# erwincoumans/tiny-differentiable-simulator

Measured on NVIDIA H100. Metric: env-steps/sec (N parallel sims), higher is better.
Workload: dtype f32 (ABA, factorisation, PGS) + f64 (kinematics, inertias, CRBA, Jacobians, LCP rhs)

## Files before the change

### tiny-differentiable-simulator_b200/csrc/tds_capi.cu

```cuda
#include <cuda_runtime.h>
#include <stdio.h>
#include <stdlib.h>
#include <string.h>

#include <algorithm>
#include <mutex>
#include <string>
#include <vector>

#include "tds_b200.h"
#include "tds_b200_model.h"
#include "tds_model.h"
#include "tds_types.h"
#include "tds_team.h"
#include "tds_tape.cuh"
#include "tds_host_io.h"

extern "C" int tds_launch_stept(const TeamModel* TM, const TeamLink* tl_dev, const DevModel* M, const SimParams* P,
                                const EnvParams* E, const StepIO* io, int mode, int use_pd, int precision,
                                char* gscratch, int use_smem, cudaStream_t stream);
extern "C" size_t tds_stept_tile_bytes(const TeamModel* TM);
extern "C" unsigned long long tds_stepr_table_owner(int dev);
extern "C" int tds_launch_stepr(const TeamModel* TM, const TeamLink* tl_host, unsigned long long token, const DevModel* M,
                                const SimParams* P, const EnvParams* E, const StepIO* io, int mode, int use_pd,
// ... 289 lines not shown
  float* S = stats + (size_t)(2 * n_obs + o) * ns + e;
  const float c = *cnt + 1.f;
  if (c == 1.f) { *mean = x; *S = 0.f; }
  else { const float m0 = *mean, m1 = m0 + (x - m0) / c; *S += (x - m0) * (x - m1); *mean = m1; }
  *cnt = c;
}
__global__ void ars_perturb_kernel(const float* __restrict__ w, const float* __restrict__ deltas, float scale,
                                   float* __restrict__ params, int n, int ns) {
  const int e = blockIdx.x * blockDim.x + threadIdx.x;
  const int p = blockIdx.y;
  if (e >= n) return;
  params[(size_t)p * ns + e] = w[p] + scale * deltas[(size_t)p * ns + e];
}
__global__ void ars_update_kernel(float* __restrict__ w, const float* __restrict__ deltas, const float* __restrict__ r_pos,
                                  const float* __restrict__ r_neg, float delta_std, float step_size, int n, int ns) {
  __shared__ float red[256];
  const int p = blockIdx.x;
  float acc = 0.f;
  for (int e = threadIdx.x; e < n; e += blockDim.x) acc += (r_pos[e] - r_neg[e]) * deltas[(size_t)p * ns + e];
  red[threadIdx.x] = acc;
  __syncthreads();
  for (int s = blockDim.x / 2; s > 0; s >>= 1) {
    if ((int)threadIdx.x < s) red[threadIdx.x] += red[threadIdx.x + s];
    __syncthreads();
  }
  if (threadIdx.x == 0) w[p] += step_size * (red[0] * delta_std / (float)n);
}
__global__ void rollout_init_kernel(float* sticky, float* total, int* steps, int n) {
  const int e = blockIdx.x * blockDim.x + threadIdx.x;
  if (e < n) { sticky[e] = 0.f; total[e] = 0.f; steps[e] = 0; }
}

}

struct tds_b200_sim {
  int device = 0;
  int n = 0, ns = 0;
  DevModel dm[3];
  DevModel dm_ad;
  char* jac_scratch = nullptr; size_t jac_scratch_bytes = 0;
  double* jac_dev = nullptr; size_t jac_dev_bytes = 0;
  int tape_cap = 4096;
  char* vjp_buf = nullptr; size_t vjp_buf_bytes = 0;
  int* vjp_flag = nullptr;
  double* vjp_g = nullptr; size_t vjp_g_bytes = 0;
  double* jvp_dev = nullptr; size_t jvp_dev_bytes = 0;
  DevModel dm_m;
  double* mass_dev = nullptr; size_t mass_dev_bytes = 0;
  ParMap par;
  double* par_dev = nullptr; size_t par_dev_bytes = 0;
  bool smem_ok[3] = {false, false, false};
  bool smem_ok_w[3] = {false, false, false};
  int kernel = 4;
  int kernel_req = 4;
  bool spec_ok = false;
  int spec_idx = -1;
  std::vector<double> model;
  bool smem_ok_r[3] = {false, false, false};
  unsigned long long table_token = 0;
  bool team_ok = false;
  bool smem_ok_t[3] = {false, false, false};
  TeamModel tm[3];
  std::vector<TeamLink> team_table;
  TeamLink* team_dev = nullptr;
  int warps_per_block[3] = {1, 1, 1};
  DevVisuals vis;
  SimParams P;
  EnvParams E;
  int precision_req = TDS_B200_PREC_AUTO;
  int precision = TDS_B200_PREC_F64;
  int n_tau = 0, n_points = 0;
  ContactCandTable cand;
  int *c_count = nullptr, *c_links = nullptr, *c_cand = nullptr;
  size_t c_count_bytes = 0, c_links_bytes = 0, c_cand_bytes = 0;
  float *q = nullptr, *qd = nullptr, *act = nullptr, *qdd = nullptr, *reward = nullptr, *done = nullptr;
  float *cdist = nullptr, *link_xf = nullptr;
  char* scratch = nullptr;
  size_t scratch_bytes = 0;
  void* stage_dev = nullptr;
  size_t stage_dev_bytes = 0;
  cudaStream_t stream = nullptr;
  int max_smem_optin = 0;
  long long* phase_clk = nullptr;
  float *rq = nullptr, *rqd = nullptr, *zero_act = nullptr, *pol_act = nullptr, *sticky = nullptr, *r_total = nullptr, *pol_params = nullptr;
  int *act_qidx = nullptr, *r_steps = nullptr;
  float* obs_stats = nullptr;
  bool act_qidx_valid = false;
  size_t pol_params_bytes = 0;
  const float* io_act_aos = nullptr; float* io_obs_aos = nullptr; float* io_obs_tail = nullptr;
  const void* zc_key[4] = {nullptr, nullptr, nullptr, nullptr};
  void* zc_dev[4] = {nullptr, nullptr, nullptr, nullptr};
  bool zc_ok = false;
  unsigned zc_calls = 0;
  const void* g_key[4] = {nullptr, nullptr, nullptr, nullptr};
  int g_seen = 0;
  cudaGraphExec_t g_exec = nullptr;
};

static void drop_host_graph(tds_b200_sim* s) {
  if (s->g_exec) { cudaGraphExecDestroy(s->g_exec); s->g_exec = nullptr; }
  s->g_seen = 0;
  s->g_key[0] = s->g_key[1] = s->g_key[2] = s->g_key[3] = nullptr;
}

static bool is_pinned(const void* p) {
  if (!p) return true;
  cudaPointerAttributes a;
  if (cudaPointerGetAttributes(&a, p) != cudaSuccess) { cudaGetLastError(); return false; }
  return a.type == cudaMemoryTypeHost;
}

static int ensure_stage(tds_b200_sim* s, size_t bytes) {
  if (bytes > s->stage_dev_bytes) {
    drop_host_graph(s);
    CUDA_TRY(grow_dev(&s->stage_dev, &s->stage_dev_bytes, bytes));
  }
  return 0;
}

static int ensure_scratch(tds_b200_sim* s, int prec) {
  const int words = s->dm[prec].w_total > s->dm[prec].x_total ? s->dm[prec].w_total : s->dm[prec].x_total;
  CUDA_TRY(grow_dev(&s->scratch, &s->scratch_bytes, (size_t)words * 4 * s->ns));
  return 0;
}

static int enter_derivative_host(tds_b200_sim* s) {
  CUDA_TRY(cudaSetDevice(s->device));
  CUDA_TRY(cudaDeviceSynchronize());
  return 0;
}


static int put_state(tds_b200_sim* s, const double* src, int dim, float* dst) {
  if (dim == 0) return 0;
  CUDA_TRY(cudaMemcpyAsync(s->stage_dev, src, sizeof(double) * s->n * dim, cudaMemcpyHostToDevice, s->stream));
  aos_to_soa_kernel<double><<<(s->n + 127) / 128, 128, 0, s->stream>>>((const double*)s->stage_dev, dim, 0, dst, dim, s->n, s->ns);
  return 0;
}

static int put_q(tds_b200_sim* s, const double* q) {
  const DevModel& M = s->dm[0];
  const size_t rows = (size_t)(M.n_q > M.n_qd ? M.n_q : M.n_qd) + s->n_points + 1;
  if (int rc = ensure_stage(s, sizeof(double) * s->n * rows)) return rc;
  return put_state(s, q, M.n_q, s->q);
}

static int put_step_inputs(tds_b200_sim* s, int use_pd, const double* q, const double* qd, const double* tau_or_action) {
  const int n_in = use_pd ? s->E.n_act : s->n_tau;
  int rc = put_q(s, q);
  if (!rc) rc = put_state(s, qd, s->dm[0].n_qd, s->qd);
  if (rc) return rc;
  if (tau_or_action) return put_state(s, tau_or_action, n_in, s->act);
  CUDA_TRY(cudaMemsetAsync(s->act, 0, sizeof(float) * s->ns * (n_in > 0 ? n_in : 1), s->stream));
  return 0;
}

static int get_state(tds_b200_sim* s, const float* src, int dim, double* dst) {
  if (dim == 0 || !dst) return 0;
  if (int rc = ensure_stage(s, sizeof(double) * s->n * dim)) return rc;
  soa_to_aos_kernel<double><<<(s->n + 127) / 128, 128, 0, s->stream>>>(src, (double*)s->stage_dev, dim, 0, dim, s->n, s->ns);
  CUDA_TRY(cudaMemcpyAsync(dst, s->stage_dev, sizeof(double) * s->n * dim, cudaMemcpyDeviceToHost, s->stream));
  CUDA_TRY(cudaStreamSynchronize(s->stream));
  return 0;
}

static int rebuild_team(tds_b200_sim* s) {
// ... 180 lines not shown
  E.auto_reset = s->E.auto_reset;
  memcpy(E.reset_q, s->E.reset_q, sizeof(E.reset_q));
  s->E = E;
  s->act_qidx_valid = false;
  return rebuild_team(s);
}

int tds_b200_set_auto_reset(tds_b200_sim* s, int enable, const double* reset_q) {
  if (!s) return -1;
  const DevModel& M = s->dm[0];
  if (enable && !reset_q) { set_err("auto-reset needs a reset pose"); return -1; }
  drop_host_graph(s);
  s->E.auto_reset = enable ? 1 : 0;
  if (reset_q)
    for (int k = 0; k < M.n_q; ++k) s->E.reset_q[k] = (float)reset_q[k];
  return 0;
}

int tds_b200_set_precision(tds_b200_sim* s, int precision) {
  if (!s || precision < TDS_B200_PREC_AUTO || precision > 2) return -1;
  drop_host_graph(s);
  s->precision_req = precision;
  s->precision = precision != TDS_B200_PREC_AUTO ? precision : (s->spec_ok ? TDS_B200_PREC_MIXED : TDS_B200_PREC_F64);
  return 0;
}

int tds_b200_param_count(const tds_b200_sim* s) { return s ? tds_param_count(&s->dm[0]) : -1; }

static int set_physical_params(tds_b200_sim* s, int k, const int* ids, const double* values, bool device, void* stream) {
  if (!s) return -1;
  if (k > 0 && !values) { set_err("physical params: null values"); return -1; }
  ParMap pm;
  const char* err = nullptr;
  if (tds_build_par_map(&s->dm[0], k, ids, &pm, &err)) { set_err(std::string("physical params: ") + err); return -2; }
  CUDA_TRY(cudaSetDevice(s->device));
  const bool same_ids = memcmp(&pm, &s->par, sizeof(pm)) == 0;
  if (!same_ids) drop_host_graph(s);
  if (k == 0) {
    s->par = pm;
    return 0;
  }
  const size_t bytes = sizeof(double) * (size_t)k * s->ns;
  if (bytes > s->par_dev_bytes) {
    drop_host_graph(s);
    CUDA_TRY(grow_dev(&s->par_dev, &s->par_dev_bytes, bytes));
    CUDA_TRY(cudaMemset(s->par_dev, 0, bytes));
  }
  if (device) {
    CUDA_TRY(cudaMemcpyAsync(s->par_dev, values, bytes, cudaMemcpyDeviceToDevice, (cudaStream_t)stream));
  } else {
    CUDA_TRY(cudaDeviceSynchronize());
    CUDA_TRY(put_rows(s->par_dev, values, k, s->n, s->ns, s->stream));
    CUDA_TRY(cudaDeviceSynchronize());
  }
  s->par = pm;
  return 0;
}

int tds_b200_set_physical_params_device(tds_b200_sim* s, int k, const int* ids, const double* values, void* stream) {
  return set_physical_params(s, k, ids, values, true, stream);
}

int tds_b200_set_physical_params_host(tds_b200_sim* s, int k, const int* ids, const double* values) {
  return set_physical_params(s, k, ids, values, false, nullptr);
}

int tds_b200_get_dims(const tds_b200_sim* s, int dims[8]) {
  if (!s) return -1;
  const DevModel& M = s->dm[0];
  dims[0] = s->n; dims[1] = s->ns; dims[2] = M.n_q; dims[3] = M.n_qd; dims[4] = s->n_tau; dims[5] = M.n_links;
  dims[6] = s->n_points; dims[7] = s->E.n_act;
  return 0;
}

int tds_b200_step_device(tds_b200_sim* s, int mode, int use_pd, const float* q_in, const float* qd_in,
                         const float* tau_or_action, float* q_out, float* qd_out, float* qdd_out, float* reward,
                         float* done, float* contact_dist, float* link_xf, void* stream) {
  if (!s) return -1;
  const int p = s->precision;
  StepIO io;
  io.q_in = q_in; io.qd_in = qd_in; io.tau_in = tau_or_action;
  io.q_out = q_out; io.qd_out = qd_out; io.qdd_out = qdd_out;
  io.reward = reward; io.done = done; io.contact_dist = contact_dist; io.link_xf = link_xf;
  io.phase_clk = s->phase_clk;
  io.act_aos = s->io_act_aos; io.obs_aos = s->io_obs_aos; io.obs_tail = s->io_obs_tail;
  io.jac = nullptr; io.jac_n_in = 0; io.jac_dir0 = 0;
  io.n = s->n; io.n_stride = s->ns;
  if (use_pd && s->E.n_act == 0) { set_err("use_pd without tds_b200_set_env"); return -3; }
  int kern = s->kernel_req;
  if (s->dm[0].world_only || mode == 3 || s->P.contact_model != 0 || s->par.n > 0) kern = 1;
  if (kern == 4 && !(s->spec_ok && tds_spec_smem_bytes(s->spec_idx, p) <= (size_t)s->max_smem_optin)) kern = 3;
  if (kern == 4) {
    s->kernel = kern;
    static const int solo = getenv("TDS_B200_DEBUG_SOLO") ? 256 : 0;
    int rcs = tds_launch_step_spec(s->spec_idx, &s->P, &s->E, &io, mode | solo, use_pd, p, (cudaStream_t)stream);
    if (rcs) set_err(std::string("specialised step launch: ") + cudaGetErrorString((cudaError_t)rcs));
    return rcs;
  }
  if (kern == 3 && !(s->team_ok && s->smem_ok_r[p])) kern = 2;
  if (kern == 2 && !s->team_ok) kern = 1;
  s->kernel = kern;
  if (kern == 3) {
    int rcr = tds_launch_stepr(&s->tm[p], s->team_table.data(), s->table_token, &s->dm[p], &s->P, &s->E, &io, mode, use_pd, p,
                               nullptr, 1, (cudaStream_t)stream);
    if (rcr) set_err(std::string("role-warp step launch: ") + cudaGetErrorString((cudaError_t)rcr));
    return rcr;
  }
  if (kern == 2) {
    const int use_smem_t = s->smem_ok_t[p] ? 1 : 0;
    if (!use_smem_t)
      CUDA_TRY(grow_dev(&s->scratch, &s->scratch_bytes, tds_stept_tile_bytes(&s->tm[p]) * ((s->n + (32 / TDS_TEAM_T) - 1) / (32 / TDS_TEAM_T))));
    int rct = tds_launch_stept(&s->tm[p], s->team_dev, &s->dm[p], &s->P, &s->E, &io, mode, use_pd, p, s->scratch, use_smem_t,
                               (cudaStream_t)stream);
    if (rct) set_err(std::string("team step launch: ") + cudaGetErrorString((cudaError_t)rct));
    return rct;
  }
  const int use_smem = s->smem_ok_w[p] ? 1 : 0;
  if (!use_smem) { int rc = ensure_scratch(s, p); if (rc) return rc; }
  ParMap pm = s->par;
  pm.values = s->par_dev; pm.grad = nullptr;
  int rc = s->par.n > 0
      ? tds_launch_stepw_par(&s->dm[p], &s->P, &s->E, &io, &pm, mode, use_pd, p, s->scratch, use_smem, s->warps_per_block[p],
                             (cudaStream_t)stream)
      : tds_launch_stepw(&s->dm[p], &s->P, &s->E, &io, mode, use_pd, p, s->scratch, use_smem, s->warps_per_block[p], (cudaStream_t)stream);
  if (rc) set_err(std::string("step launch: ") + cudaGetErrorString((cudaError_t)rc));
  return rc;
}

int tds_b200_jacobian_dims(const tds_b200_sim* s, int mode, int use_pd, int dims[2]) {
  if (!s || !dims) return -1;
  const DevModel& M = s->dm[0];
  dims[0] = mode == TDS_B200_MODE_FD ? M.n_qd : M.n_q + M.n_qd;
  dims[1] = M.n_q + M.n_qd + (use_pd ? s->E.n_act + 3 : s->n_tau);
  return 0;
}

struct JvpTangents { const double* t_in; const double* t_par; int m; bool mass = false; const TdsKinCall* kin = nullptr; };

static size_t lane_arena_bytes(const tds_b200_sim* s, const DevModel& M) {
  return (size_t)(s->n + 31) / 32 * (size_t)M.x_total * 32 * 4;
}

static int dir_chunk(const tds_b200_sim* s) {
  const size_t chunk = ((size_t)2 << 30) / lane_arena_bytes(s, s->dm_ad);
  return (int)(chunk < 1 ? 1 : (chunk > 65535 ? 65535 : chunk));
}

static int jacobian_run(tds_b200_sim* s, int mode, int use_pd, const float* q, const float* qd, const float* tau_or_action,
                        double* jac, void* stream, bool params, const JvpTangents* jv = nullptr) {
  int dims[2];
  tds_b200_jacobian_dims(s, mode, use_pd, dims);
  const int n_dirs = jv ? jv->m : (params ? s->par.n : dims[1]), dir_base = (params && !jv) ? dims[1] : 0;
  StepIO io;
  memset(&io, 0, sizeof(io));
  io.q_in = q; io.qd_in = qd; io.tau_in = tau_or_action;
  io.jac = jac; io.jac_n_in = n_dirs;
  io.n = s->n; io.n_stride = s->ns;
  ParMap pmv = s->par;
  pmv.values = s->par_dev; pmv.grad = nullptr;
  const ParMap* pm = s->par.n > 0 ? &pmv : nullptr;
  const int chunk = std::min(dir_chunk(s), n_dirs);
  CUDA_TRY(grow_dev(&s->jac_scratch, &s->jac_scratch_bytes, lane_arena_bytes(s, s->dm_ad) * chunk));
  for (int d0 = 0; d0 < n_dirs; d0 += chunk) {
    io.jac_dir0 = dir_base + d0;
    const int nd = n_dirs - d0 < chunk ? n_dirs - d0 : chunk;
    int rc = (jv && jv->kin) ? tds_launch_kin_jvp(&s->dm_ad, &io, jv->kin, jv->t_in, jv->m, nd, s->jac_scratch, (cudaStream_t)stream)
           : (jv && jv->mass) ? tds_launch_mass_jvp(&s->dm_ad, &io, pm, jv->t_in, jv->t_par, jv->m, nd, s->jac_scratch, (cudaStream_t)stream)
// ... 726 lines not shown
  return 0;
}

int tds_b200_env_set_obs_stats(tds_b200_sim* s, float* stats) {
  if (!s) return -1;
  s->obs_stats = stats;
  return 0;
}

int tds_b200_env_rollout_device(tds_b200_sim* s, const float* policy, int n_params, int rollout_length, float shift,
                                float* total_rewards, int* steps, void* stream) {
  if (!s || !policy || !total_rewards || !steps) return -1;
  if (s->E.n_act == 0) { set_err("rollout without tds_b200_set_env"); return -3; }
  const DevModel& M = s->dm[0];
  if (n_params != s->E.n_act * (M.n_q + M.n_qd) + s->E.n_act) { set_err("policy size must be n_act * (n_q + n_qd) + n_act"); return -2; }
  CUDA_TRY(cudaSetDevice(s->device));
  int rc = ensure_env_layer(s);
  if (rc) return rc;
  cudaStream_t sm = stream ? (cudaStream_t)stream : s->stream;
  const int T = 128, B = (s->n + T - 1) / T;
  rollout_init_kernel<<<B, T, 0, sm>>>(s->sticky, total_rewards, steps, s->n);
  const int saved_auto = s->E.auto_reset;
  s->E.auto_reset = 0;
  for (int r = 0; r < rollout_length && rc == 0; ++r) {
    policy_linear_kernel<<<dim3(B, s->E.n_act), T, 0, sm>>>(s->q, s->qd, policy, s->pol_act, M.n_q, M.n_qd, s->E.n_act, s->n, s->ns);
    if (s->obs_stats) obs_stat_push_kernel<<<dim3(B, M.n_q + M.n_qd), T, 0, sm>>>(s->q, s->qd, s->obs_stats, M.n_q, M.n_qd, s->n, s->ns);
    rc = tds_b200_step_device(s, TDS_B200_MODE_FULL, 1, s->q, s->qd, s->pol_act, s->q, s->qd, nullptr, s->reward, s->done, nullptr,
                              nullptr, sm);
    rollout_accum_kernel<<<B, T, 0, sm>>>(s->reward, s->done, shift, s->sticky, total_rewards, steps, s->n);
  }
  s->E.auto_reset = saved_auto;
  if (rc) return rc;
  CUDA_TRY(cudaGetLastError());
  return 0;
}

int tds_b200_env_rollout_host(tds_b200_sim* s, const double* policy, int n_params, int rollout_length, double shift,
                              const double* noise, double noise_amp, unsigned long long seed, int settle_steps,
                              double* total_rewards, int* steps) {
  if (!s || !policy) return -1;
  CUDA_TRY(cudaSetDevice(s->device));
  int rc = ensure_env_layer(s);
  if (rc) return rc;
  const int n = s->n, ns = s->ns, na = s->E.n_act;
  cudaStream_t sm = s->stream;
  const size_t rows = (size_t)n_params > (size_t)na ? (size_t)n_params : (size_t)na;
  CUDA_TRY(grow_dev(&s->pol_params, &s->pol_params_bytes, sizeof(float) * rows * ns));
  rc = ensure_stage(s, sizeof(double) * (size_t)n * rows);
  if (!rc && noise) rc = put_state(s, noise, na, s->pol_params);
  if (!rc) rc = tds_b200_env_reset_device(s, nullptr, noise ? s->pol_params : nullptr, (float)noise_amp, seed, settle_steps, sm);
  if (!rc) rc = put_state(s, policy, n_params, s->pol_params);
  if (!rc) rc = tds_b200_env_rollout_device(s, s->pol_params, n_params, rollout_length, (float)shift, s->r_total, s->r_steps, sm);
  if (rc) return rc;
  std::vector<float> tot(n);
  CUDA_TRY(cudaMemcpyAsync(tot.data(), s->r_total, sizeof(float) * n, cudaMemcpyDeviceToHost, sm));
  if (steps) CUDA_TRY(cudaMemcpyAsync(steps, s->r_steps, sizeof(int) * n, cudaMemcpyDeviceToHost, sm));
  CUDA_TRY(cudaStreamSynchronize(sm));
  if (total_rewards) for (int i = 0; i < n; ++i) total_rewards[i] = (double)tot[i];
  return 0;
}

int tds_b200_get_precision(const tds_b200_sim* s) { return s ? s->precision : -1; }

const char* tds_b200_kernel_name(const tds_b200_sim* s) {
  static const char* names[5] = {"", "tds_stepw_kernel (common frame, lane per environment)",
                                 "tds_stept_kernel (lane team per environment)", "tds_stepr_kernel (warp per tree role)",
                                 "tds_step_spec_kernel (warp per tree role, model-specialised)"};
  return (s && s->kernel >= 0 && s->kernel <= 4) ? names[s->kernel] : "";
}

int tds_b200_debug_phase_clocks(tds_b200_sim* s, int enable, long long* out_host, int cap_warps) {
  if (!s) return -1;
  const int nw = s->ns / (32 / TDS_TEAM_T);
  if (enable && !s->phase_clk) {
    CUDA_TRY(cudaMalloc((void**)&s->phase_clk, sizeof(long long) * 16 * nw));
    CUDA_TRY(cudaMemset(s->phase_clk, 0, sizeof(long long) * 16 * nw));
  }
  if (out_host && s->phase_clk) {
    CUDA_TRY(cudaDeviceSynchronize());
    CUDA_TRY(cudaMemcpy(out_host, s->phase_clk, sizeof(long long) * 16 * (nw < cap_warps ? nw : cap_warps), cudaMemcpyDeviceToHost));
  }
  if (!enable && s->phase_clk) { cudaFree(s->phase_clk); s->phase_clk = nullptr; }
  return nw;
}

void* tds_b200_stream(tds_b200_sim* s) { return s ? (void*)s->stream : nullptr; }
float* tds_b200_env_q(tds_b200_sim* s) { return s ? s->q : nullptr; }
float* tds_b200_env_qd(tds_b200_sim* s) { return s ? s->qd : nullptr; }

int tds_b200_env_step_host(tds_b200_sim* s, const float* actions, float* obs, float* rewards, float* dones) {
  if (!s || !actions) return -1;
  CUDA_TRY(cudaSetDevice(s->device));
  const DevModel& M = s->dm[0];
  const int n = s->n, ns = s->ns, na = s->E.n_act, nobs = M.n_q + M.n_qd;
  const size_t in_b = sizeof(float) * (size_t)n * na, obs_b = sizeof(float) * (size_t)n * nobs;
  const bool packed = obs && rewards == obs + (size_t)n * nobs && dones == rewards + n;
  int rc = ensure_stage(s, in_b + obs_b + sizeof(float) * 2 * (size_t)n);
  if (rc) return rc;
  float* d_in = (float*)s->stage_dev;
  float* d_obs = (float*)((char*)s->stage_dev + in_b);
  cudaStream_t sm = s->stream;
  const int T = 128, B = (n + T - 1) / T;
  const bool direct = s->kernel_req == 4 && s->spec_ok && s->P.contact_model == 0 && s->par.n == 0 && tds_spec_smem_bytes(s->spec_idx, s->precision) <= (size_t)s->max_smem_optin;
  auto enqueue = [&]() -> int {
    CUDA_TRY(cudaMemcpyAsync(d_in, actions, in_b, cudaMemcpyHostToDevice, sm));
    if (direct) {
      s->io_act_aos = d_in; s->io_obs_aos = obs ? d_obs : nullptr; s->io_obs_tail = (obs && packed) ? d_obs + (size_t)n * nobs : nullptr;
    } else aos_to_soa_kernel<float><<<B, T, 0, sm>>>(d_in, na, 0, s->act, na, n, ns);
    int r = tds_b200_step_device(s, TDS_B200_MODE_FULL, 1, s->q, s->qd, s->act, s->q, s->qd, nullptr, s->reward, s->done,
                                 nullptr, nullptr, sm);
    s->io_act_aos = nullptr; s->io_obs_aos = nullptr; s->io_obs_tail = nullptr;
    if (r) return r;
    if (obs && direct) {
      CUDA_TRY(cudaMemcpyAsync(obs, d_obs, obs_b + (packed ? sizeof(float) * 2 * (size_t)n : 0), cudaMemcpyDeviceToHost, sm));
    } else if (obs) {
      pack_env_out_kernel<<<B, T, 0, sm>>>(s->q, s->qd, s->reward, s->done, d_obs, M.n_q, M.n_qd, n, ns, packed ? 1 : 0);
      CUDA_TRY(cudaMemcpyAsync(obs, d_obs, obs_b + (packed ? sizeof(float) * 2 * (size_t)n : 0), cudaMemcpyDeviceToHost, sm));
    }
    if (!packed) {
      if (rewards) CUDA_TRY(cudaMemcpyAsync(rewards, s->reward, sizeof(float) * n, cudaMemcpyDeviceToHost, sm));
      if (dones) CUDA_TRY(cudaMemcpyAsync(dones, s->done, sizeof(float) * n, cudaMemcpyDeviceToHost, sm));
    }
    return 0;
  };
  static const bool no_zero_copy = getenv("TDS_B200_NO_ZEROCOPY") != nullptr;
  if (direct && !s->phase_clk && !no_zero_copy) {
    void *da = nullptr, *dob = nullptr, *dr = nullptr, *dd = nullptr;
    bool ok;
    if ((++s->zc_calls & 63u) != 0 && s->zc_key[0] == actions && s->zc_key[1] == obs && s->zc_key[2] == rewards && s->zc_key[3] == dones) {
      ok = s->zc_ok;
      da = s->zc_dev[0]; dob = s->zc_dev[1]; dr = s->zc_dev[2]; dd = s->zc_dev[3];
    } else {
      ok = is_pinned(actions) && is_pinned(obs) && is_pinned(rewards) && is_pinned(dones);
      ok = ok && cudaHostGetDevicePointer(&da, (void*)actions, 0) == cudaSuccess;
      if (ok && obs) ok = cudaHostGetDevicePointer(&dob, obs, 0) == cudaSuccess;
      if (ok && rewards) ok = cudaHostGetDevicePointer(&dr, rewards, 0) == cudaSuccess;
      if (ok && dones) ok = cudaHostGetDevicePointer(&dd, dones, 0) == cudaSuccess;
      if (!ok) cudaGetLastError();
      s->zc_key[0] = actions; s->zc_key[1] = obs; s->zc_key[2] = rewards; s->zc_key[3] = dones;
      s->zc_dev[0] = da; s->zc_dev[1] = dob; s->zc_dev[2] = dr; s->zc_dev[3] = dd;
      s->zc_ok = ok;
    }
    if (ok) {
      s->io_act_aos = (const float*)da; s->io_obs_aos = (float*)dob; s->io_obs_tail = nullptr;
      rc = tds_b200_step_device(s, TDS_B200_MODE_FULL, 1, s->q, s->qd, s->act, s->q, s->qd, nullptr, dr ? (float*)dr : s->reward,
                                dd ? (float*)dd : s->done, nullptr, nullptr, sm);
      s->io_act_aos = nullptr; s->io_obs_aos = nullptr;
      if (rc) return rc;
      CUDA_TRY(cudaStreamSynchronize(sm));
      CUDA_TRY(cudaGetLastError());
      return 0;
    }
  }
  const void* key[4] = {actions, obs, rewards, dones};
  const bool same = s->g_key[0] == key[0] && s->g_key[1] == key[1] && s->g_key[2] == key[2] && s->g_key[3] == key[3];
  if (s->g_exec && s->kernel == 3 && tds_stepr_table_owner(s->device) != s->table_token) drop_host_graph(s);
  if (same && s->g_exec) {
    CUDA_TRY(cudaGraphLaunch(s->g_exec, sm));
  } else if (same && s->g_seen >= 2 && !s->phase_clk && is_pinned(actions) && is_pinned(obs) && is_pinned(rewards) && is_pinned(dones)) {
    cudaGraph_t g = nullptr;
    CUDA_TRY(cudaStreamBeginCapture(sm, cudaStreamCaptureModeThreadLocal));
    rc = enqueue();
    cudaError_t ce = cudaStreamEndCapture(sm, &g);
    if (rc || ce != cudaSuccess) {
      if (g) cudaGraphDestroy(g);
      cudaGetLastError();
// ... 214 lines not shown
```

### tiny-differentiable-simulator_b200/csrc/tds_steps.cu

```cuda
#include <cuda_runtime.h>
#include <stdlib.h>

#include "tds_wcommon.cuh"
#include "tds_team.h"
#include "generated/spec_laikago.h"
#include "generated/spec_ant.h"

namespace tdss {
using namespace tds;
using namespace tdsw;

#ifndef TDS_DENSE_MAX_CAND
#define TDS_DENSE_MAX_CAND 8
#endif
constexpr int TT = TDS_TEAM_T;
constexpr int ST = 32;

template <int V> struct IC { static constexpr int value = V; };
#define CI(...) (IC<(__VA_ARGS__)>::value)
#define CD(...) ([]() { constexpr double cd_v_ = (__VA_ARGS__); return cd_v_; }())
#define CDOT3(ax, ay, az, v)                                                                                            \
  ([&]() {                                                                                                              \
    using T_ = decltype((v).x);                                                                                         \
    constexpr double a_ = (ax), b_ = (ay), c_ = (az);                                                                   \
// ... 145 lines not shown
  }
  return true;
}
template <class SP> __host__ __device__ constexpr bool trunk_direct() {
  if (!trunk_is_chain<SP>() || SP::FLOATING) return false;
  for (int k = 0; k < SP::N_TRUNK; ++k) {
    if (SP::L_FLAGS[0][k] & TDS_LF_FIXED) return false;
    if (SP::L_SD[0][k][0] != 0.0 || SP::L_SD[0][k][1] != 0.0) return false;
    if (k < SP::N_TRUNK - 1 && (!trunk_massless<SP>(k) || SP::L_ACC[0][k] >= 0 || SP::L_XW[0][k] >= 0)) return false;
  }
  return true;
}
template <class SP> constexpr TrunkTab<SP> make_trunk() {
  TrunkTab<SP> t{};
  for (int k = 0; k < SP::N_TRUNK; ++k) {
    const double* b = SP::L_RBIC[0][k];
    t.fixed[k] = (SP::L_FLAGS[0][k] & TDS_LF_FIXED) ? 1 : 0;
    t.massless[k] = (b[0] == 0.0 && b[4] == 0.0 && b[5] == 0.0 && b[6] == 0.0 && b[7] == 0.0 && b[8] == 0.0 && b[9] == 0.0) ? 1 : 0;
    t.rbi_slot[k] = trunk_rbi_slot<SP>(k);
    t.acc[k] = SP::L_ACC[0][k]; t.ldof[k] = SP::L_LDOF[0][k]; t.qdidx[k] = SP::L_QDIDX[0][k]; t.xw[k] = SP::L_XW[0][k];
    t.sd[k][0] = (float)SP::L_SD[0][k][0]; t.sd[k][1] = (float)SP::L_SD[0][k][1];
  }
  return t;
}
template <class SP> __device__ const TrunkTab<SP>& trunk_tab();

template <class SP> struct CandTab {
  static constexpr int NC = SP::N_CAND > 0 ? SP::N_CAND : 1;
  int owner[NC], own[NC];
};
template <class SP> constexpr CandTab<SP> make_cand() {
  CandTab<SP> t{};
  for (int g = 0; g < SP::N_CAND; ++g) {
    t.owner[g] = SP::CAND_OWNER[g];
    t.own[g] = (SP::CAND_OWNER[g] == 0 && SP::CAND_LPT[g] < Cls<SP>::n_pts_trunk()) ? 0 : 1;
  }
  return t;
}
template <class SP> __device__ const CandTab<SP>& cand_tab();

template <class SP, typename RA, typename RC, typename RS> struct Lay {
  static constexpr int RAW = sizeof(RA) / 4, RCW = sizeof(RC) / 4, RSW = sizeof(RS) / 4;
  static constexpr int NTD = SP::N_TD, NTRI = NTD * (NTD + 1) / 2, NOD = SP::N_OD_MAX;
  static constexpr int O = 0;
  static constexpr int RB = O + 4 * RCW;
  static constexpr int XWW = ev(12 * RCW + 12 * RAW);
  static constexpr int XW = RB + 10 * RCW;
  static constexpr int TS = XW + (SP::N_XW_TEAM + 1) * XWW;
  static constexpr int TLW = ev(14 * RAW);
  static constexpr int TL = TS + SP::N_TRUNK * 6 * RCW;
  static constexpr int TLR = ev(TL + SP::N_TRUNK * TLW);
  static constexpr int TKS = ev(TLR + trunk_rbi_slot<SP>(SP::N_TRUNK) * 10 * RCW);
  static constexpr int TQD = ev(TKS + 3 * SP::N_TRUNK);
  static constexpr int ACC_IC = ev(27 * RAW);
  static constexpr int ACCW = ev(ACC_IC + 10 * RCW);
  static constexpr int ACC = ev(TQD + NTD);
  static constexpr int PW = ev(NTRI * RSW);
  static constexpr int CONW = ev((3 * (NOD + NTD) + 9) * RSW);
  static constexpr int ACC_SZ = cmax(cmax(TT * cmax(SP::N_ATT, 1) * ACCW, TT * PW), cmax(SP::N_CAND, 1) * CONW);
  static constexpr int LT = ACC + ACC_SZ;
  static constexpr int CON = ACC;
  static constexpr int ZT = ev(LT + NTRI * RSW);
  static constexpr int WO = ev(ZT + NTD * RSW);
  static constexpr int ASTG = ev(WO + TT * NOD * RSW);
  static constexpr int XS = ev(ASTG + SP::N_ACT);
  static constexpr int FLG = ev(XS + (SP::N_CAND > TDS_DENSE_MAX_CAND ? 3 * SP::N_CAND * RSW : 0));
  static constexpr int SHARED = ev(FLG + 2 * TT + 2);
  static constexpr int PRIV = ev(cmax(SP::KMAX - SP::N_TRUNK, 1) * 10 * RCW);
  static constexpr int TOTAL = SHARED + TT * PRIV;
};

template <typename T> TDS_D T* sp(char* base, int lane, int word) {
  return (sizeof(T) == 4) ? ((T*)base) + (size_t)word * ST + lane : ((T*)base) + (size_t)(word >> 1) * ST + lane;
}
template <typename T> TDS_D T negz() { return T(-0.0); }
template <typename T> TDS_D Abi<T> abi_nz() {
  Abi<T> a; const T z = negz<T>();
  a.I = {z, z, z, z, z, z}; a.M = a.I;
  a.H.xx = a.H.xy = a.H.xz = a.H.yx = a.H.yy = a.H.yz = a.H.zx = a.H.zy = a.H.zz = z;
  return a;
}
template <typename T> TDS_D Sv<T> sv_nz() { Sv<T> s; const T z = negz<T>(); s.top = v3<T>(z, z, z); s.bot = s.top; return s; }
template <typename T> TDS_D Rbi<T> rbi_nz() { Rbi<T> r; const T z = negz<T>(); r.m = z; r.h = v3<T>(z, z, z); r.I = {z, z, z, z, z, z}; return r; }

template <class SP, typename RA, typename RC, typename RS, int VAR>
TDS_D void tile_body(char* const smem, const SimParams& P, const EnvParams& E, const StepIO& io, const int mode, const int use_pd,
                     const int role, const int tile, const int tid) {
  using L = Lay<SP, RA, RC, RS>;
  using C = Cls<SP>;
  static_assert(C::uniform(), "the subtrees of the model are not one structural class (use the table-driven kernel)");
  constexpr bool XOUT = VAR == 0, HOSTIO = VAR == 2;
  constexpr int RAW = L::RAW, RCW = L::RCW;
  constexpr int NT = SP::N_TRUNK, NTD = SP::N_TD, NLOC = SP::N_LOC[0];
  constexpr int NOD = SP::N_OD[0], NODA = cmax(NOD, 1), NTDA = cmax(NTD, 1), NTRI = L::NTRI, NTRIA = cmax(NTRI, 1);
  constexpr int NPO = C::n_pts_own(), NPOA = cmax(NPO, 1), NPTR = C::n_pts_trunk(), NPTRA = cmax(NPTR, 1);
  constexpr int NACCA = cmax(SP::N_ACC, 1), NXLA = cmax(SP::N_XW_LANE, 1), NATT = cmax(SP::N_ATT, 1);
  constexpr bool FLOAT = SP::FLOATING != 0;
  const int lane = tid & 31;
  const int env = tile * 32 + lane;
  const bool live = env < io.n;
  const int e = live ? env : io.n - 1;
  const int ns = io.n_stride;
  const LegTab<SP>& LG = leg_tab<SP>(role);
  char* const priv = smem + (size_t)(L::SHARED + role * L::PRIV) * ST * 4;
  int phase_id = 0;
#define TDSS_PHASE() do { if (io.phase_clk && lane == 0 && tile * 32 < io.n_stride) io.phase_clk[((size_t)tile * TT + role) * 16 + phase_id] = clock64(); ++phase_id; } while (0)
#define TDSS_STAMP(slot) do { if (io.phase_clk && lane == 0 && tile * 32 < io.n_stride) io.phase_clk[((size_t)tile * TT + role) * 16 + (slot)] = clock64(); } while (0)
  TDSS_PHASE();
  auto xw_rc = [&](int slot) { return sp<RC>(smem, lane, L::XW + slot * L::XWW); };
  auto xw_ra = [&](int slot) { return sp<RA>(smem, lane, L::XW + slot * L::XWW + 12 * RCW); };
  auto tl_rbi_slot = [&](int slot) { return sp<RC>(smem, lane, L::TLR + slot * 10 * RCW); };
  auto tl_u = [&](int k) { return sp<RA>(smem, lane, L::TL + k * L::TLW); };
  auto tl_v = [&](int k) { return sp<RA>(smem, lane, L::TL + k * L::TLW + 8 * RAW); };
  auto ts_S = [&](int k) { return sp<RC>(smem, lane, L::TS + k * 6 * RCW); };
  float* const tqd = sp<float>(smem, lane, L::TQD);
  unsigned* const flg = sp<unsigned>(smem, lane, L::FLG);

  float qv[SP::KMAX], qdv[SP::KMAX], tauv[SP::KMAX];
  float bq[7], bqd[6];
  sfor<NT, NLOC>([&](auto Kc) {
    constexpr int k = decltype(Kc)::value;
    if constexpr (!(C::flags(k) & TDS_LF_FIXED)) {
      qv[k] = io.q_in[(size_t)LG.qidx[k - NT] * ns + e];
      qdv[k] = io.qd_in[(size_t)LG.qdidx[k - NT] * ns + e];
      tauv[k] = 0.f;
    }
  });
  if (role == 0) {
    sfor<0, NT>([&](auto Kc) {
      constexpr int k = decltype(Kc)::value;
      if constexpr (!(SP::L_FLAGS[0][k] & TDS_LF_FIXED)) {
        qv[k] = io.q_in[(size_t)CI(SP::L_QIDX[0][k]) * ns + e];
        qdv[k] = io.qd_in[(size_t)CI(SP::L_QDIDX[0][k]) * ns + e];
        tauv[k] = 0.f;
      }
    });
    if constexpr (FLOAT) {
#pragma unroll
      for (int k = 0; k < 7; ++k) bq[k] = io.q_in[(size_t)k * ns + e];
#pragma unroll
      for (int k = 0; k < 6; ++k) bqd[k] = io.qd_in[(size_t)k * ns + e];
    }
  }
  constexpr int NACT_TILE = 32 * SP::N_ACT, AREG = (NACT_TILE + 32 * TT - 1) / (32 * TT);
  float areg[AREG];
  if constexpr (HOSTIO) {
    const float* const ta = io.act_aos + (size_t)tile * NACT_TILE;
    const int rows = io.n - tile * 32;
    const int valid = (rows < 32 ? rows : 32) * SP::N_ACT;
#pragma unroll
    for (int j = 0; j < AREG; ++j) {
      const int idx = tid + 32 * TT * j;
      areg[j] = idx < valid ? ta[idx] : 0.f;
    }
  }
  float* const astg = (float*)smem + (size_t)L::ASTG * ST;
  const float* const act_p = HOSTIO ? astg + lane * SP::N_ACT : io.tau_in + e;
  const size_t act_s = HOSTIO ? (size_t)1 : (size_t)ns;
  auto pd_torques = [&]() {
    sfor<NT, NLOC>([&](auto Kc) {
      constexpr int k = decltype(Kc)::value;
      if constexpr (!(C::flags(k) & TDS_LF_FIXED) && SP::L_ACT[0][k] >= 0) {
        const int a = LG.act[k - NT];
        float act = act_p[(size_t)a * act_s];
        act = fmaxf(fminf(act, E.action_limit), -E.action_limit);
        const float q_des = E.initial_poses[a] + act;
// ... 1136 lines not shown
      constexpr int k0 = k_of_q<SP, 0>(0), k2 = k_of_q<SP, 0>(2), k3 = k_of_q<SP, 0>(3), k4 = k_of_q<SP, 0>(4);
      if constexpr (!FLOAT && k0 >= 0 && k0 < NT && k2 >= 0 && k2 < NT && k3 >= 0 && k3 < NT && k4 >= 0 && k4 < NT) {
        const float x = qv[k0], z = qv[k2];
        const float upz = cosf(qv[k3]) * cosf(qv[k4]);
        done = (upz < 0.6f) || (z < 0.2f);
        rew = done ? 0.f : x;
        if (io.reward && live) io.reward[e] = rew;
      }
    } else if (E.reward_kind == 3) {
      constexpr int k0 = k_of_q<SP, 0>(0), k2 = k_of_q<SP, 0>(2);
      if constexpr (!FLOAT && k0 >= 0 && k0 < NT && k2 >= 0 && k2 < NT) {
        done = qv[k2] < 0.26f;
        rew = done ? 0.f : qdv[k0];
        if (io.reward && live) io.reward[e] = rew;
      }
    } else if (E.reward_kind == 2) {
      if constexpr (FLOAT) {
        const float x = bq[4], z = bq[6];
        done = ((float)up_z < 0.6f) || (z < 0.2f);
        rew = done ? 0.f : x;
        if (io.reward && live) io.reward[e] = rew;
      }
    }
    if (io.done && E.reward_kind && live) io.done[e] = done ? 1.f : 0.f;
    if constexpr (HOSTIO) if (io.obs_tail && live) { io.obs_tail[e] = rew; io.obs_tail[io.n + e] = done ? 1.f : 0.f; }
    flg[(2 * TT) * ST] = done ? 1u : 0u;
  }
  __syncthreads();
  const bool reset = (flg[(2 * TT) * ST] != 0u) && E.auto_reset;
  float* const ostg = (float*)smem + (size_t)L::ACC * ST;
  static_assert(!HOSTIO || (SP::N_Q + SP::N_QD) <= L::ACC_SZ, "observation staging does not fit the reused region");
  if (live) {
    sfor<NT, NLOC>([&](auto Kc) {
      constexpr int k = decltype(Kc)::value;
      if constexpr (!(C::flags(k) & TDS_LF_FIXED)) {
        const int qi = LG.qidx[k - NT], qdi = LG.qdidx[k - NT];
        const float qo = reset ? E.reset_q[qi] : qv[k], qdo = reset ? 0.f : qdv[k];
        io.q_out[(size_t)qi * ns + e] = qo;
        io.qd_out[(size_t)qdi * ns + e] = qdo;
        if constexpr (HOSTIO) { float* o = ostg + lane * (SP::N_Q + SP::N_QD); o[qi] = qo; o[SP::N_Q + qdi] = qdo; }
      }
    });
    if (role == 0) {
      sfor<0, NT>([&](auto Kc) {
        constexpr int k = decltype(Kc)::value;
        if constexpr (!(SP::L_FLAGS[0][k] & TDS_LF_FIXED)) {
          const float qo = reset ? E.reset_q[CI(SP::L_QIDX[0][k])] : qv[k], qdo = reset ? 0.f : qdv[k];
          io.q_out[(size_t)CI(SP::L_QIDX[0][k]) * ns + e] = qo;
          io.qd_out[(size_t)CI(SP::L_QDIDX[0][k]) * ns + e] = qdo;
          if constexpr (HOSTIO) { float* o = ostg + lane * (SP::N_Q + SP::N_QD); o[CI(SP::L_QIDX[0][k])] = qo; o[SP::N_Q + CI(SP::L_QDIDX[0][k])] = qdo; }
        }
      });
      if constexpr (FLOAT) {
#pragma unroll
        for (int k = 0; k < 7; ++k) {
          const float qo = reset ? E.reset_q[k] : bq[k];
          io.q_out[(size_t)k * ns + e] = qo;
          if constexpr (HOSTIO) ostg[lane * (SP::N_Q + SP::N_QD) + k] = qo;
        }
#pragma unroll
        for (int k = 0; k < 6; ++k) {
          const float qdo = reset ? 0.f : bqd[k];
          io.qd_out[(size_t)k * ns + e] = qdo;
          if constexpr (HOSTIO) ostg[lane * (SP::N_Q + SP::N_QD) + SP::N_Q + k] = qdo;
        }
      }
    }
  }
  if constexpr (HOSTIO) {
    if (io.obs_aos) {
      __syncthreads();
      constexpr int NOBS = SP::N_Q + SP::N_QD;
      const int rows = io.n - tile * 32;
      const int valid = (rows < 32 ? rows : 32) * NOBS;
      float* const dst = io.obs_aos + (size_t)tile * 32 * NOBS;
      if (valid == 32 * NOBS && (NOBS % 4) == 0) {
        for (int i = tid; i < 8 * NOBS; i += 32 * TT) ((float4*)dst)[i] = ((const float4*)ostg)[i];
      } else {
        for (int i = tid; i < valid; i += 32 * TT) dst[i] = ostg[i];
      }
    }
  }
  TDSS_PHASE();
#undef TDSS_PHASE
#undef TDSS_STAMP
}

template <class SP, typename RA, typename RC, typename RS, int VAR, int TPC>
__global__ void __launch_bounds__(32 * TDS_TEAM_T * TPC, TPC == 1 ? 2 : 1)
tds_step_spec_kernel(const __grid_constant__ SimParams P, const __grid_constant__ EnvParams E, const StepIO io, const int mode_flags,
                     const int use_pd) {
  extern __shared__ __align__(16) char smem_raw[];
  const int warp = __shfl_sync(0xffffffffu, (int)(threadIdx.x >> 5), 0);
  const int role = warp % TDS_TEAM_T, sub = warp / TDS_TEAM_T;
  if ((mode_flags & 256) && role != 0) return;
#ifndef TDS_STEPS_KERNEL_ONLY
  if (mode_flags & 512) asm volatile("griddepcontrol.launch_dependents;");
  asm volatile("griddepcontrol.wait;" ::: "memory");
#endif
  char* const smem = smem_raw + (size_t)sub * ((size_t)Lay<SP, RA, RC, RS>::TOTAL * 32 * 4);
  tile_body<SP, RA, RC, RS, VAR>(smem, P, E, io, mode_flags & 255, use_pd, role, (int)blockIdx.x * TPC + sub,
                                 (int)threadIdx.x - sub * 32 * TDS_TEAM_T);
#ifndef TDS_STEPS_KERNEL_ONLY
  if (!(mode_flags & 512)) asm volatile("griddepcontrol.launch_dependents;");
#endif
}

#ifndef TDS_STEPS_KERNEL_ONLY
template <class SP> struct SpecHost {
  static bool matches(const DevModel* D, const EnvParams* E) {
    if (D->n_links != SP::N_LINKS || D->n_q != SP::N_Q || D->n_qd != SP::N_QD || D->floating != SP::FLOATING) return false;
    if (E->n_act != 0) {
      if (E->n_act != SP::N_ACT) return false;
      for (int a = 0; a < SP::N_ACT; ++a) if (E->act_link[a] != SP::ACT_LINK[a]) return false;
    }
    auto trunk_q = [](int q) { const int k = k_of_q<SP, 0>(q); return k >= 0 && k < SP::N_TRUNK; };
    if (E->reward_kind == 1 && (SP::FLOATING || !trunk_q(0) || !trunk_q(2) || !trunk_q(3) || !trunk_q(4))) return false;
    if (E->reward_kind == 2 && !SP::FLOATING) return false;
    if (E->reward_kind == 3 && (SP::FLOATING || !trunk_q(0) || !trunk_q(2))) return false;
    return true;
  }
  static bool same_model(const double* model, int n_model, const double* mine, int n_mine) {
    const int n_dyn = TDSM_HEADER + TDSM_BASE + SP::N_LINKS * TDSM_LINK + SP::N_GEOMS * TDSM_GEOM;
    if (n_dyn > n_mine || n_dyn > n_model) return false;
    for (int i = 0; i < n_dyn; ++i) {
      if (i == TDSM_H_NVIS) continue;
      if (!(model[i] == mine[i])) return false;
    }
    return true;
  }
  static size_t smem_bytes(int precision) {
    if (precision == 0) return (size_t)Lay<SP, float, double, float>::TOTAL * 32 * 4;
    if (precision == 1) return (size_t)Lay<SP, double, double, double>::TOTAL * 32 * 4;
    return (size_t)Lay<SP, float, float, float>::TOTAL * 32 * 4;
  }
  static int launch(const SimParams* P, const EnvParams* E, const StepIO* io, int mode, int use_pd, int precision, cudaStream_t stream) {
    const int tiles = (io->n + 31) / 32;
    const size_t smem1 = smem_bytes(precision);
    cudaError_t err = cudaSuccess;
    int dev_ = 0; cudaGetDevice(&dev_);
    static int sm_count[64] = {0};
    if (!sm_count[dev_ & 63]) cudaDeviceGetAttribute(&sm_count[dev_ & 63], cudaDevAttrMultiProcessorCount, dev_);
    static const int tpc_env = getenv("TDS_B200_TPC") ? atoi(getenv("TDS_B200_TPC")) : 0;
    static const bool pdl = getenv("TDS_B200_PDL") ? atoi(getenv("TDS_B200_PDL")) != 0 : false;
    int tpc = 1;
    if (tpc_env == -1) tpc = (tiles > 2 * sm_count[dev_ & 63] && 2 * smem1 <= 227 * 1024) ? 2 : 1;
    if (tpc_env == 2) tpc = 2 * smem1 <= 227 * 1024 ? 2 : 1;
#define TDSS_LAUNCH(RA, RC, RS, VAR, TPC)                                                               \
  do {                                                                                                  \
    auto k = tds_step_spec_kernel<SP, RA, RC, RS, VAR, TPC>;                                            \
    const size_t smem = smem1 * TPC;                                                                    \
    static bool attr_set_dev[64] = {false}; bool& attr_set = attr_set_dev[dev_ & 63];  \
    if (!attr_set && smem > 48 * 1024) {                                                                \
      err = cudaFuncSetAttribute(k, cudaFuncAttributeMaxDynamicSharedMemorySize, (int)smem);            \
       \
      if (err == cudaSuccess) err = cudaFuncSetAttribute(k, cudaFuncAttributePreferredSharedMemoryCarveout, cudaSharedmemCarveoutMaxShared); \
      if (err == cudaSuccess) attr_set = true;                                                          \
    }                                                                                                   \
    if (err == cudaSuccess) {                                                                           \
      cudaLaunchConfig_t cfg = {};                                                                      \
      cfg.gridDim = dim3((tiles + TPC - 1) / TPC); cfg.blockDim = dim3(32 * TDS_TEAM_T * TPC);          \
      cfg.dynamicSmemBytes = smem; cfg.stream = stream;                                                 \
      cudaLaunchAttribute at[1];                                                                        \
      at[0].id = cudaLaunchAttributeProgrammaticStreamSerialization;                                    \
      at[0].val.programmaticStreamSerializationAllowed = 1;                                             \
      cfg.attrs = at; cfg.numAttrs = pdl ? 1 : 0;                                                       \
      const int mode_k = mode | ((pdl && tiles <= sm_count[dev_ & 63]) ? 512 : 0);                      \
      err = cudaLaunchKernelEx(&cfg, k, *P, *E, *io, mode_k, use_pd);                                   \
    }                                                                                                   \
  } while (0)
    const int var = ((mode & 255) == 0 || io->link_xf || io->contact_dist || io->qdd_out) ? 0 : ((io->act_aos && use_pd) ? 2 : 1);
    if (var != 2 && io->act_aos) return (int)cudaErrorInvalidValue;
#define TDSS_PREC(VAR, TPC)                                                      \
  do {                                                                           \
    if (precision == 0) TDSS_LAUNCH(float, double, float, VAR, TPC);             \
    else if (precision == 1) TDSS_LAUNCH(double, double, double, VAR, TPC);      \
    else TDSS_LAUNCH(float, float, float, VAR, TPC);                             \
  } while (0)
    if (var == 0) TDSS_PREC(0, 1);
#ifdef TDS_B200_WITH_TPC2
    else if (var == 1 && tpc == 2 && precision != 1) { if (precision == 0) TDSS_LAUNCH(float, double, float, 1, 2); else TDSS_LAUNCH(float, float, float, 1, 2); }
    else if (var == 2 && tpc == 2 && precision != 1) { if (precision == 0) TDSS_LAUNCH(float, double, float, 2, 2); else TDSS_LAUNCH(float, float, float, 2, 2); }
#endif
    else if (var == 1) TDSS_PREC(1, 1);
    else TDSS_PREC(2, 1);
#undef TDSS_PREC
#undef TDSS_LAUNCH
    return (int)err;
  }
};
#endif

}

#define TDS_SPEC_TABLES(SP, sym)                                                                                          \
  namespace tdss {                                                                                                        \
  __constant__ LegTab<SP> c_legs_##sym[TDS_TEAM_T] = {make_leg<SP>(0), make_leg<SP>(1), make_leg<SP>(2), make_leg<SP>(3)}; \
  template <> __device__ __forceinline__ const LegTab<SP>& leg_tab<SP>(int role) { return c_legs_##sym[role]; }            \
  __constant__ TrunkTab<SP> c_trunk_##sym = make_trunk<SP>();                                                             \
  template <> __device__ __forceinline__ const TrunkTab<SP>& trunk_tab<SP>() { return c_trunk_##sym; }                    \
  __constant__ CandTab<SP> c_cand_##sym = make_cand<SP>();                                                                \
  template <> __device__ __forceinline__ const CandTab<SP>& cand_tab<SP>() { return c_cand_##sym; }                       \
  }
TDS_SPEC_TABLES(SpecLaikago, laikago)
TDS_SPEC_TABLES(SpecAnt, ant)

#ifndef TDS_STEPS_KERNEL_ONLY
static const double k_spec_laikago_model[] = {
#include "generated/laikago_model.inc"
};
static const double k_spec_ant_model[] = {
#include "generated/ant_model.inc"
};

extern "C" int tds_spec_find(const double* model, int n_model, const DevModel* D, const EnvParams* E) {
  using namespace tdss;
  if (SpecHost<SpecLaikago>::same_model(model, n_model, k_spec_laikago_model, (int)(sizeof(k_spec_laikago_model) / sizeof(double))) &&
      SpecHost<SpecLaikago>::matches(D, E)) return 0;
  if (SpecHost<SpecAnt>::same_model(model, n_model, k_spec_ant_model, (int)(sizeof(k_spec_ant_model) / sizeof(double))) &&
      SpecHost<SpecAnt>::matches(D, E)) return 1;
  return -1;
}

extern "C" size_t tds_spec_smem_bytes(int spec, int precision) {
  using namespace tdss;
  return spec == 0 ? SpecHost<SpecLaikago>::smem_bytes(precision) : SpecHost<SpecAnt>::smem_bytes(precision);
}

extern "C" const char* tds_spec_name(int spec) { return spec == 0 ? "laikago" : (spec == 1 ? "ant" : ""); }

extern "C" int tds_launch_step_spec(int spec, const SimParams* P, const EnvParams* E, const StepIO* io, int mode, int use_pd,
                                    int precision, cudaStream_t stream) {
  using namespace tdss;
  if (spec == 0) return SpecHost<SpecLaikago>::launch(P, E, io, mode, use_pd, precision, stream);
  if (spec == 1) return SpecHost<SpecAnt>::launch(P, E, io, mode, use_pd, precision, stream);
  return (int)cudaErrorInvalidValue;
}
#endif
```

Measured before the change: 332.5 million.

## Enable PDL by default with early dependent launch and input L2 prefetch

Programmatic dependent launch is now always on. Dependents are released early whenever the whole grid fits in one wave, computed through an occupancy query. Before griddepcontrol.wait, each thread prefetches its tile's q/qd/tau rows into L2 so the next step's input loads overlap the previous kernel's tail. When there are at most one CTA per SM, dynamic shared memory is padded to half the SM's capacity to control co-residency. Optional globaltimer stamps are also added for device-side phase profiling, at the cost of extra complexity and a possible early-launch hazard if inputs are not ready.

```diff
diff --git a/tiny-differentiable-simulator_b200/csrc/tds_capi.cu b/tiny-differentiable-simulator_b200/csrc/tds_capi.cu
--- a/tiny-differentiable-simulator_b200/csrc/tds_capi.cu
+++ b/tiny-differentiable-simulator_b200/csrc/tds_capi.cu
@@ -395,6 +395,7 @@
   cudaStream_t stream = nullptr;
   int max_smem_optin = 0;
   long long* phase_clk = nullptr;
+  long long* phase_clk_dev = nullptr;
   float *rq = nullptr, *rqd = nullptr, *zero_act = nullptr, *pol_act = nullptr, *sticky = nullptr, *r_total = nullptr, *pol_params = nullptr;
   int *act_qidx = nullptr, *r_steps = nullptr;
   float* obs_stats = nullptr;
@@ -741,7 +742,7 @@
   io.q_in = q_in; io.qd_in = qd_in; io.tau_in = tau_or_action;
   io.q_out = q_out; io.qd_out = qd_out; io.qdd_out = qdd_out;
   io.reward = reward; io.done = done; io.contact_dist = contact_dist; io.link_xf = link_xf;
-  io.phase_clk = s->phase_clk;
+  io.phase_clk = s->phase_clk_dev ? s->phase_clk_dev : s->phase_clk;
   io.act_aos = s->io_act_aos; io.obs_aos = s->io_obs_aos; io.obs_tail = s->io_obs_tail;
   io.jac = nullptr; io.jac_n_in = 0; io.jac_dir0 = 0;
   io.n = s->n; io.n_stride = s->ns;
@@ -1634,6 +1635,12 @@
   }
   if (!enable && s->phase_clk) { cudaFree(s->phase_clk); s->phase_clk = nullptr; }
   return nw;
+}
+
+int tds_b200_debug_phase_clocks_device(tds_b200_sim* s, long long* dev) {
+  if (!s) return -1;
+  s->phase_clk_dev = dev;
+  return 0;
 }
 
 void* tds_b200_stream(tds_b200_sim* s) { return s ? (void*)s->stream : nullptr; }
diff --git a/tiny-differentiable-simulator_b200/csrc/tds_steps.cu b/tiny-differentiable-simulator_b200/csrc/tds_steps.cu
--- a/tiny-differentiable-simulator_b200/csrc/tds_steps.cu
+++ b/tiny-differentiable-simulator_b200/csrc/tds_steps.cu
@@ -251,6 +251,16 @@
 }
 template <typename T> TDS_D Sv<T> sv_nz() { Sv<T> s; const T z = negz<T>(); s.top = v3<T>(z, z, z); s.bot = s.top; return s; }
 template <typename T> TDS_D Rbi<T> rbi_nz() { Rbi<T> r; const T z = negz<T>(); r.m = z; r.h = v3<T>(z, z, z); r.I = {z, z, z, z, z, z}; return r; }
+
+TDS_D long long global_ns() {
+#ifdef TDS_STEPS_KERNEL_ONLY
+  return 0;
+#else
+  unsigned long long t;
+  asm volatile("mov.u64 %0, %%globaltimer;" : "=l"(t));
+  return (long long)t;
+#endif
+}
 
 template <class SP, typename RA, typename RC, typename RS, int VAR>
 TDS_D void tile_body(char* const smem, const SimParams& P, const EnvParams& E, const StepIO& io, const int mode, const int use_pd,
@@ -1553,8 +1563,22 @@
     }
   }
   TDSS_PHASE();
+  if (io.phase_clk && lane == 0 && tile * 32 < io.n_stride) io.phase_clk[((size_t)tile * TT + role) * 16 + 15] = global_ns();
 #undef TDSS_PHASE
 #undef TDSS_STAMP
+}
+
+template <class SP, int VAR> TDS_D void prefetch_tile_rows(const StepIO& io, const int use_pd, const int tile, const int tid) {
+  constexpr int NA = VAR == 2 ? 0 : SP::N_ACT, NTAU = VAR == 2 ? 0 : SP::N_QD - (SP::FLOATING ? 6 : 0);
+  const int n_in = io.tau_in ? (use_pd ? NA : NTAU) : 0;
+  const size_t col = (size_t)tile * 32;
+  const float* row = nullptr;
+  if (tid < SP::N_Q) row = io.q_in + (size_t)tid * io.n_stride;
+  else if (tid < SP::N_Q + SP::N_QD) row = io.qd_in + (size_t)(tid - SP::N_Q) * io.n_stride;
+  else if (tid < SP::N_Q + SP::N_QD + n_in) row = io.tau_in + (size_t)(tid - SP::N_Q - SP::N_QD) * io.n_stride;
+#ifndef TDS_STEPS_KERNEL_ONLY
+  if (row) asm volatile("prefetch.global.L2 [%0];" :: "l"(row + col));
+#endif
 }
 
 template <class SP, typename RA, typename RC, typename RS, int VAR, int TPC>
@@ -1565,13 +1589,19 @@
   const int warp = __shfl_sync(0xffffffffu, (int)(threadIdx.x >> 5), 0);
   const int role = warp % TDS_TEAM_T, sub = warp / TDS_TEAM_T;
   if ((mode_flags & 256) && role != 0) return;
+  const int tile = (int)blockIdx.x * TPC + sub, tid = (int)threadIdx.x - sub * 32 * TDS_TEAM_T;
+  char* const smem = smem_raw + (size_t)sub * ((size_t)Lay<SP, RA, RC, RS>::TOTAL * 32 * 4);
+  long long* const gstamp = (io.phase_clk && (tid & 31) == 0 && tile * 32 < io.n_stride) ? io.phase_clk + ((size_t)tile * TDS_TEAM_T + role) * 16 : nullptr;
+  if (gstamp && role == 0) gstamp[14] = global_ns();
 #ifndef TDS_STEPS_KERNEL_ONLY
   if (mode_flags & 512) asm volatile("griddepcontrol.launch_dependents;");
+#endif
+  prefetch_tile_rows<SP, VAR>(io, use_pd, tile, tid);
+#ifndef TDS_STEPS_KERNEL_ONLY
   asm volatile("griddepcontrol.wait;" ::: "memory");
 #endif
-  char* const smem = smem_raw + (size_t)sub * ((size_t)Lay<SP, RA, RC, RS>::TOTAL * 32 * 4);
-  tile_body<SP, RA, RC, RS, VAR>(smem, P, E, io, mode_flags & 255, use_pd, role, (int)blockIdx.x * TPC + sub,
-                                 (int)threadIdx.x - sub * 32 * TDS_TEAM_T);
+  if (gstamp && role != 0) gstamp[14] = global_ns();
+  tile_body<SP, RA, RC, RS, VAR>(smem, P, E, io, mode_flags & 255, use_pd, role, tile, tid);
 #ifndef TDS_STEPS_KERNEL_ONLY
   if (!(mode_flags & 512)) asm volatile("griddepcontrol.launch_dependents;");
 #endif
@@ -1612,8 +1642,9 @@
     int dev_ = 0; cudaGetDevice(&dev_);
     static int sm_count[64] = {0};
     if (!sm_count[dev_ & 63]) cudaDeviceGetAttribute(&sm_count[dev_ & 63], cudaDevAttrMultiProcessorCount, dev_);
+    static int smem_per_sm[64] = {0};
+    if (!smem_per_sm[dev_ & 63]) cudaDeviceGetAttribute(&smem_per_sm[dev_ & 63], cudaDevAttrMaxSharedMemoryPerMultiprocessor, dev_);
     static const int tpc_env = getenv("TDS_B200_TPC") ? atoi(getenv("TDS_B200_TPC")) : 0;
-    static const bool pdl = getenv("TDS_B200_PDL") ? atoi(getenv("TDS_B200_PDL")) != 0 : false;
     int tpc = 1;
     if (tpc_env == -1) tpc = (tiles > 2 * sm_count[dev_ & 63] && 2 * smem1 <= 227 * 1024) ? 2 : 1;
     if (tpc_env == 2) tpc = 2 * smem1 <= 227 * 1024 ? 2 : 1;
@@ -1622,21 +1653,27 @@
     auto k = tds_step_spec_kernel<SP, RA, RC, RS, VAR, TPC>;                                            \
     const size_t smem = smem1 * TPC;                                                                    \
     static bool attr_set_dev[64] = {false}; bool& attr_set = attr_set_dev[dev_ & 63];  \
-    if (!attr_set && smem > 48 * 1024) {                                                                \
-      err = cudaFuncSetAttribute(k, cudaFuncAttributeMaxDynamicSharedMemorySize, (int)smem);            \
+    static int ctas_per_sm_dev[64] = {0}; int& ctas_per_sm = ctas_per_sm_dev[dev_ & 63];              \
+    const size_t smem_one = smem > (size_t)smem_per_sm[dev_ & 63] / 2 ? smem : (size_t)smem_per_sm[dev_ & 63] / 2; \
+    if (!attr_set && smem_one > 48 * 1024) {                                                            \
+      err = cudaFuncSetAttribute(k, cudaFuncAttributeMaxDynamicSharedMemorySize, (int)smem_one);        \
        \
       if (err == cudaSuccess) err = cudaFuncSetAttribute(k, cudaFuncAttributePreferredSharedMemoryCarveout, cudaSharedmemCarveoutMaxShared); \
       if (err == cudaSuccess) attr_set = true;                                                          \
     }                                                                                                   \
+    if (err == cudaSuccess && !ctas_per_sm)                                                             \
+      err = cudaOccupancyMaxActiveBlocksPerMultiprocessor(&ctas_per_sm, k, 32 * TDS_TEAM_T * TPC, smem); \
     if (err == cudaSuccess) {                                                                           \
+      const int ctas = (tiles + TPC - 1) / TPC;                                                         \
+      const bool one_per_sm = ctas <= sm_count[dev_ & 63];                                              \
       cudaLaunchConfig_t cfg = {};                                                                      \
-      cfg.gridDim = dim3((tiles + TPC - 1) / TPC); cfg.blockDim = dim3(32 * TDS_TEAM_T * TPC);          \
-      cfg.dynamicSmemBytes = smem; cfg.stream = stream;                                                 \
+      cfg.gridDim = dim3(ctas); cfg.blockDim = dim3(32 * TDS_TEAM_T * TPC);                             \
+      cfg.dynamicSmemBytes = one_per_sm ? smem_one : smem; cfg.stream = stream;                         \
       cudaLaunchAttribute at[1];                                                                        \
       at[0].id = cudaLaunchAttributeProgrammaticStreamSerialization;                                    \
       at[0].val.programmaticStreamSerializationAllowed = 1;                                             \
-      cfg.attrs = at; cfg.numAttrs = pdl ? 1 : 0;                                                       \
-      const int mode_k = mode | ((pdl && tiles <= sm_count[dev_ & 63]) ? 512 : 0);                      \
+      cfg.attrs = at; cfg.numAttrs = 1;                                                                 \
+      const int mode_k = mode | (one_per_sm || ctas <= ctas_per_sm * sm_count[dev_ & 63] ? 512 : 0);   \
       err = cudaLaunchKernelEx(&cfg, k, *P, *E, *io, mode_k, use_pd);                                   \
     }                                                                                                   \
   } while (0)
```

New measurement: 364.6 million (median of 6 runs). 1.1x the previous value.
